# Mesoptier/ray-marching

Measured on AMD Instinct MI355X. Metric: Mpixels/s at 1920x1080, 256-step march, 32-node SDF, higher is better.
Workload: dtype f32; 1 GPU; 1920x1080, g32 (31 commands / 111 words), 256 max steps, 16 rays/px, RGBA32F out; camera=still, kernel=0, specialized_kernel=True, jit_from_disk_cache=True, frames_in_flight=4

## Files before the change

### ray-marching_amd/csrc/rm_jit.h

```cpp
#pragma once
#include <atomic>
#include <chrono>
#include <condition_variable>
#include <cstdio>
#include <cstdlib>
#include <cstring>
#include <dlfcn.h>
#include <sys/stat.h>
#include <unistd.h>
#include <map>
#include <memory>
#include <mutex>
#include <string>
#include <thread>
#include <vector>

#include "rm_device.h"
#include "rm_units.h"

namespace rmjit {

#include "generated/rm_jit_sources.inc"

constexpr uint32_t kMaxRecords = 255u;

struct Rtc {
    typedef struct _hiprtcProgram* Program;
    int (*CreateProgram)(Program*, const char*, const char*, int, const char* const*, const char* const*) = nullptr;
    int (*CompileProgram)(Program, int, const char* const*) = nullptr;
    int (*GetProgramLogSize)(Program, size_t*) = nullptr;
    int (*GetProgramLog)(Program, char*) = nullptr;
    int (*GetCodeSize)(Program, size_t*) = nullptr;
    int (*GetCode)(Program, char*) = nullptr;
// ... 36 lines not shown
        DestroyProgram = reinterpret_cast<decltype(DestroyProgram)>(sym("hiprtcDestroyProgram"));
        if (!all) { handle = nullptr; return; }
        Version = reinterpret_cast<decltype(Version)>(dlsym(handle, "hiprtcVersion"));
        int major = 0, minor = 0;
        if (Version) (void)Version(&major, &minor);
        Dl_info info;
        std::memset(&info, 0, sizeof info);
        (void)dladdr(reinterpret_cast<void*>(CreateProgram), &info);
        identity = std::string(info.dli_fname ? info.dli_fname : "?") + ":" + std::to_string(major) + "." + std::to_string(minor);
    }
};

inline std::string structure_key(const std::vector<RmRecord>& rec) {
    std::string k;
    k.reserve(rec.size() * 2);
    for (const RmRecord& r : rec) {
        k.push_back("PSBCLXM?"[RM_OP_KIND(r.op)]);
        k.push_back("pusixy??"[RM_OP_MODE(r.op)]);
        if (RM_OP_KIND(r.op) == RM_KIND_POP && RM_OP_MODE(r.op) == RM_MODE_SMOOTH && !(r.p[0] == r.p[0] && std::fabs(r.p[0]) < 1.0e30f)) k.push_back('!');
    }
    return k;
}

inline bool can_specialise(const std::vector<RmRecord>& rec) { return !rec.empty() && rec.size() <= kMaxRecords; }

inline int jit_knob(const char* name, int dflt) {
    const char* v = std::getenv(name);
    return v ? std::atoi(v) : dflt;
}

enum : int { PRUNE_NONE = 0, PRUNE_LATTICE = 1, PRUNE_BLEND = 2 };
enum : int { KERNEL_WITH_STATS = 0x100, PRUNE_KIND_MASK = 0xFF };

inline bool generate_scene_code(const std::vector<RmRecord>& rec, int prune, int T, std::string* out) {
    const int count_mode = (prune && T == 1) ? jit_knob("RM_JIT_PRUNE_STATS", 0) : 0;
    const char* counted = count_mode == 1 ? " n_eval += 1u;" : "";
    const int sched_every = T == 1 ? 4 : 2;
    const bool sub_tests = jit_knob("RM_JIT_SUB_TESTS", 1) != 0 && T == 1;
    const bool fence = T == 4;
    std::vector<RmUnit> units;
    if (prune == PRUNE_LATTICE && !rm_lattice_units(rec, &units)) return false;
    if (prune == PRUNE_BLEND && !rm_blend_units(rec, &units)) return false;
    std::vector<int> unit_at(rec.size(), -1);
    for (size_t u = 0; u < units.size(); u++) unit_at[(size_t)units[u].first] = (int)u;

    std::string s;
    char line[1024];
    s += "namespace rmk {\ntemplate <bool FAST>\n";
    if (T == 1) {
        s += "RM_DEV float map_scene_spec(LdsF lp, float qx, float qy, float qz, unsigned long long need, unsigned long long live, SqrtGuard& tiny, uint32_t& n_eval) {\n";
        if (prune) s += "    const float inf = __uint_as_float(0x7F800000u);\n";
        s += "    const float x0 = qx, y0 = qy, z0 = qz;\n";
    } else {
        s += "RM_DEV void map_scene_taps(LdsF lp, float cx, float cy, float cz, unsigned long long need, unsigned long long live, SqrtGuard& tiny, float (&f)[4]) {\n";
        if (prune) s += "    const float inf = __uint_as_float(0x7F800000u);\n";
        s += "    const float e = 0.0001f;\n";
        s += "    const float x0_0 = cx + e, x0_1 = cx - e, x0_2 = cx - e, x0_3 = cx + e;\n";
        s += "    const float y0_0 = cy - e, y0_1 = cy - e, y0_2 = cy + e, y0_3 = cy + e;\n";
        s += "    const float z0_0 = cz - e, z0_1 = cz + e, z0_2 = cz - e, z0_3 = cz + e;\n";
    }
    auto V = [&](int w, int t) { char b[32]; if (T == 1) std::snprintf(b, sizeof b, "v%d", w); else std::snprintf(b, sizeof b, "v%d_%d", w, t); return std::string(b); };
    auto P = [&](int c, int t) {
        char b[96];
        if (T == 1) std::snprintf(b, sizeof b, "x%d, y%d, z%d", c, c, c);
        else std::snprintf(b, sizeof b, "x%d_%d, y%d_%d, z%d_%d", c, t, c, t, c, t);
        return std::string(b);
    };
    auto leaf_fn = [](uint32_t kind) -> const char* {
        return kind == RM_KIND_SPHERE ? "spec_sphere<FAST>" : kind == RM_KIND_BOX ? "spec_box<FAST>" : kind == RM_KIND_CYLINDER ? "spec_cylinder<FAST>"
             : kind == RM_KIND_PLANE ? "spec_plane" : nullptr;
    };
    auto leaf_expr = [&](size_t i, int c, int t) {
        const uint32_t kind = RM_OP_KIND(rec[i].op);
        char b[256];
        if (kind == RM_KIND_PLANE) std::snprintf(b, sizeof b, "%s(lp + %u, %s)", leaf_fn(kind), (unsigned)i * 8u, P(c, t).c_str());
        else std::snprintf(b, sizeof b, "%s(lp + %u, %s, tiny)", leaf_fn(kind), (unsigned)i * 8u, P(c, t).c_str());
        return std::string(b);
// ... 2 lines not shown
    auto emit_smooth = [&](const char* decl, int w, unsigned koff, const std::vector<std::string>& a, const std::vector<std::string>& b, const char* ind) {
        if (T == 1) {
            std::snprintf(line, sizeof line, "%s%s%s = spec_smooth_union(lp + %u, %s, %s, live);\n", ind, decl, V(w, 0).c_str(), koff, a[0].c_str(), b[0].c_str());
            s += line;
            return;
        }
        if (decl[0]) {
            std::snprintf(line, sizeof line, "%sfloat %s, %s, %s, %s;\n", ind, V(w, 0).c_str(), V(w, 1).c_str(), V(w, 2).c_str(), V(w, 3).c_str());
            s += line;
        }
        std::snprintf(line, sizeof line,
                      "%s{ const float sa[4] = {%s, %s, %s, %s}, sb[4] = {%s, %s, %s, %s}; float so[4];\n"
                      "%s  spec_smooth_union4(lp + %u, sa, sb, live, so); %s = so[0]; %s = so[1]; %s = so[2]; %s = so[3]; }\n",
                      ind, a[0].c_str(), a[1].c_str(), a[2].c_str(), a[3].c_str(), b[0].c_str(), b[1].c_str(), b[2].c_str(), b[3].c_str(),
                      ind, koff, V(w, 0).c_str(), V(w, 1).c_str(), V(w, 2).c_str(), V(w, 3).c_str());
        s += line;
    };
    auto names = [&](int w) { std::vector<std::string> n; for (int t = 0; t < T; t++) n.push_back(V(w, t)); return n; };

    std::vector<int> stack;
    std::vector<int> pos;
    pos.push_back(0);
    int nv = 0, np = 0, leaves = 0;
    auto after_leaf = [&](bool is_plane) {
        if (fence && !is_plane) s += "    guard_fence(tiny);\n";
        if (sched_every > 0 && ++leaves % sched_every == 0) s += "    __builtin_amdgcn_sched_barrier(0);\n";
    };
    auto emit_plain = [&](size_t first, size_t last, const char* ind) -> bool {
        for (size_t i = first; i <= last; i++) {
            const uint32_t kind = RM_OP_KIND(rec[i].op), mode = RM_OP_MODE(rec[i].op);
            const unsigned off = (unsigned)i * 8u;
            if (kind == RM_KIND_MATERIAL) return false;
            if (kind == RM_KIND_XFORM) {
                const int c = pos.back();
                if ((mode & 1u) == 0u) {
                    const int n = ++np;
                    for (int t = 0; t < T; t++) {
                        char cx[24], cy[24], cz[24], nx[24], ny[24], nz[24];
                        auto nm = [&](char* b, char a, int q) { if (T == 1) std::snprintf(b, 24, "%c%d", a, q); else std::snprintf(b, 24, "%c%d_%d", a, q, t); };
                        nm(cx, 'x', c); nm(cy, 'y', c); nm(cz, 'z', c); nm(nx, 'x', n); nm(ny, 'y', n); nm(nz, 'z', n);
                        if (mode == RM_XF_T_PUSH)
                            std::snprintf(line, sizeof line, "%sconst float %s = %s - lp[%u], %s = %s - lp[%u], %s = %s - lp[%u];\n", ind, nx, cx, off, ny, cy, off + 1u, nz, cz, off + 2u);
                        else if (mode == RM_XF_R_PUSH)
                            std::snprintf(line, sizeof line, "%sfloat %s = %s, %s = %s, %s = %s; xf_rotate_conj(lp[%u], lp[%u], lp[%u], lp[%u], %s, %s, %s);\n",
                                          ind, nx, cx, ny, cy, nz, cz, off, off + 1u, off + 2u, off + 3u, nx, ny, nz);
                        else
                            std::snprintf(line, sizeof line, "%sconst float %s = %s / lp[%u], %s = %s / lp[%u], %s = %s / lp[%u];\n", ind, nx, cx, off, ny, cy, off, nz, cz, off);
                        s += line;
                    }
                    pos.push_back(n);
                } else {
                    if (pos.size() < 2 || stack.empty()) return false;
                    pos.pop_back();
                    if (mode == RM_XF_S_POP) {
                        const int a = stack.back(); stack.pop_back();
                        const int w = nv++;
                        for (int t = 0; t < T; t++) {
                            std::snprintf(line, sizeof line, "%sconst float %s = %s * lp[%u];\n", ind, V(w, t).c_str(), V(a, t).c_str(), off);
                            s += line;
                        }
                        stack.push_back(w);
                    }
                }
                continue;
            }
            const char* op = op_name(mode);
            if (kind == RM_KIND_POP) {
                if (stack.size() < 2 || mode == RM_MODE_PUSH) return false;
                const int b = stack.back(); stack.pop_back();
                const int a = stack.back(); stack.pop_back();
                const int w = nv++;
                if (mode == RM_MODE_SMOOTH) {
                    emit_smooth("const float ", w, off, names(a), names(b), ind);
                } else {
                    if (!op) return false;
                    for (int t = 0; t < T; t++) {
                        std::snprintf(line, sizeof line, "%sconst float %s = %s(%s, %s);\n", ind, V(w, t).c_str(), op, V(a, t).c_str(), V(b, t).c_str());
                        s += line;
                    }
                }
                stack.push_back(w);
                continue;
            }
            if (!leaf_fn(kind) || mode == RM_MODE_SMOOTH || (mode != RM_MODE_PUSH && !op)) return false;
            int a = -1;
            if (mode != RM_MODE_PUSH) {
                if (stack.empty()) return false;
                a = stack.back(); stack.pop_back();
            }
            const int w = nv++;
            for (int t = 0; t < T; t++) {
                if (mode == RM_MODE_PUSH) std::snprintf(line, sizeof line, "%sconst float %s = %s;%s\n", ind, V(w, t).c_str(), leaf_expr(i, pos.back(), t).c_str(), counted);
                else std::snprintf(line, sizeof line, "%sconst float %s = %s(%s, %s);%s\n", ind, V(w, t).c_str(), op, V(a, t).c_str(), leaf_expr(i, pos.back(), t).c_str(), counted);
                s += line;
            }
            stack.push_back(w);
            after_leaf(kind == RM_KIND_PLANE);
        }
        return true;
    };

    std::vector<int> group_first(units.size(), 0);
    if (jit_knob("RM_JIT_UNIT_GROUPS", 1) != 0) {
        auto flows = [&](size_t u) {
            const RmUnit& q = units[u];
            if (q.kind == RM_UNIT_OPAQUE || q.leaf < 0) return false;
            const uint32_t m = q.k_rec >= 0 ? (uint32_t)RM_MODE_SMOOTH : RM_OP_MODE(rec[(size_t)q.first].op);
            if (m == RM_MODE_PUSH || (m == RM_MODE_INTER && q.kind == RM_UNIT_LEAF)) return false;
            return true;
        };
        auto pushes = [&](size_t u) {
            const RmUnit& q = units[u];
            if (q.kind == RM_UNIT_OPAQUE || q.leaf < 0 || q.k_rec >= 0 || q.first != q.last) return false;
            return RM_OP_MODE(rec[(size_t)q.first].op) == RM_MODE_PUSH;
        };
        for (size_t u = 0; u < units.size();) {
            if (!flows(u) && !(pushes(u) && u + 1 < units.size() && flows(u + 1) && units[u + 1].first == units[u].last + 1)) { u++; continue; }
// ... 12 lines not shown
    int group_left = 0, group_value = -1;

    for (size_t i = 0; i < rec.size();) {
        const int ui = unit_at[i];
        if (ui < 0) {
            if (!emit_plain(i, i, "    ")) return false;
            i++;
            continue;
        }
        const RmUnit& u = units[(size_t)ui];
        const uint32_t kind = RM_OP_KIND(rec[i].op), mode = RM_OP_MODE(rec[i].op);
        const int c = pos.back();
        if (group_left == 0 && group_first[(size_t)ui] != 0) {
            const bool fresh = mode == RM_MODE_PUSH && u.k_rec < 0;
            if (!fresh && stack.empty()) return false;
            group_left = group_first[(size_t)ui];
            group_value = nv++;
            for (int t = 0; t < T; t++) {
                std::snprintf(line, sizeof line, "    float %s = %s;\n", V(group_value, t).c_str(), fresh ? "inf" : V(stack.back(), t).c_str());
                s += line;
            }
            uint32_t mask = 0u;
            for (int k = 0; k < group_left; k++) mask |= 1u << ((ui + k) & 31);
            std::snprintf(line, sizeof line, "    { const uint32_t wg = unit_word(need, %du);\n    if ((wg & 0x%xu) != 0u) {\n", ui, mask);
            s += line;
        }
        char guard[64];
        if (group_left != 0) std::snprintf(guard, sizeof guard, "unit_in_word(wg, %du)", ui);
        else std::snprintf(guard, sizeof guard, "unit_needed(need, %du)", ui);
        auto close_group = [&]() {
            if (group_left == 0 || --group_left != 0) return;
            for (int t = 0; t < T; t++) { std::snprintf(line, sizeof line, "        %s = %s;\n", V(group_value, t).c_str(), V(stack.back(), t).c_str()); s += line; }
            s += "    } }\n";
            stack.back() = group_value;
        };
        if (u.kind == RM_UNIT_OPAQUE) {
            if (stack.empty()) return false;
            const int a = stack.back();
            const int w = nv++;
            for (int t = 0; t < T; t++) { std::snprintf(line, sizeof line, "    float %s = %s;\n", V(w, t).c_str(), V(a, t).c_str()); s += line; }
            std::snprintf(line, sizeof line, "    if (unit_needed(need, %du)) {\n", ui);
            s += line;
            const size_t depth0 = stack.size();
            if (!emit_plain((size_t)u.first, (size_t)u.last, "        ") || stack.size() != depth0) return false;
            for (int t = 0; t < T; t++) { std::snprintf(line, sizeof line, "        %s = %s;\n", V(w, t).c_str(), V(stack.back(), t).c_str()); s += line; }
            s += "    }\n";
            stack.back() = w;
            i = (size_t)u.last + 1u;
            continue;
        }
        const bool with_smooth = u.k_rec >= 0;
        const uint32_t eff_mode = with_smooth ? (uint32_t)RM_MODE_SMOOTH : mode;
        int a = -1;
        if (eff_mode != RM_MODE_PUSH) {
            if (stack.empty()) return false;
            a = stack.back(); stack.pop_back();
        }
        const int w = nv++;
        const bool to_inf = eff_mode == RM_MODE_PUSH || (eff_mode == RM_MODE_INTER && u.kind == RM_UNIT_LEAF);
        for (int t = 0; t < T; t++) {
            if (to_inf) std::snprintf(line, sizeof line, "    float %s = inf;\n", V(w, t).c_str());
            else std::snprintf(line, sizeof line, "    float %s = %s;\n", V(w, t).c_str(), V(a, t).c_str());
            s += line;
        }
        std::snprintf(line, sizeof line, "    if (%s) {%s\n", guard, counted);
        s += line;
        const unsigned off = (unsigned)i * 8u;
        if (with_smooth) {
            std::vector<std::string> lv;
            for (int t = 0; t < T; t++) lv.push_back(leaf_expr(i, c, t));
            emit_smooth("", w, (unsigned)u.k_rec * 8u, names(a), lv, "        ");
        } else if (eff_mode == RM_MODE_SUB && sub_tests && (kind == RM_KIND_SPHERE || kind == RM_KIND_BOX)) {
            if (kind == RM_KIND_SPHERE)
                std::snprintf(line, sizeof line, "        const float a = spec_sphere_a(lp + %u, %s);\n        if (spec_sub_sphere_near(live, lp + %u, a, %s)) %s = vmax_negb(%s, spec_sphere_v<FAST>(lp + %u, a, tiny));\n",
                              off, P(c, 0).c_str(), off, V(a, 0).c_str(), V(w, 0).c_str(), V(a, 0).c_str(), off);
            else
                std::snprintf(line, sizeof line, "        const SpecBox b = spec_box_a(lp + %u, %s);\n        if (spec_sub_box_near(live, b.a, %s)) %s = vmax_negb(%s, spec_box_v<FAST>(b, tiny));\n",
                              off, P(c, 0).c_str(), V(a, 0).c_str(), V(w, 0).c_str(), V(a, 0).c_str());
            s += line;
        } else {
            const char* op = op_name(eff_mode);
            if (eff_mode != RM_MODE_PUSH && !op) return false;
            for (int t = 0; t < T; t++) {
                if (eff_mode == RM_MODE_PUSH) std::snprintf(line, sizeof line, "        %s = %s;\n", V(w, t).c_str(), leaf_expr(i, c, t).c_str());
                else std::snprintf(line, sizeof line, "        %s = %s(%s, %s);\n", V(w, t).c_str(), op, V(a, t).c_str(), leaf_expr(i, c, t).c_str());
                s += line;
            }
        }
        s += "    }\n";
        stack.push_back(w);
        after_leaf(false);
        close_group();
        i = (size_t)u.last + 1u;
    }
    if (stack.empty() || group_left != 0) return false;
    if (T == 1) {
        std::snprintf(line, sizeof line, "    return %s;\n}\n}  // namespace rmk\n", V(stack.back(), 0).c_str());
        s += line;
    } else {
        for (int t = 0; t < 4; t++) {
            std::snprintf(line, sizeof line, "    f[%d] = %s;\n", t, V(stack.back(), t).c_str());
            s += line;
        }
        s += "}\n}  // namespace rmk\n";
    }
    *out = std::move(s);
    return true;
}


inline bool generate_material_walk(const std::vector<RmRecord>& mrec, std::string* out) {
    std::string s;
    char line[768];
    s += "namespace rmk {\n";
    s += "template <bool FAST>\n";
    s += "RM_DEV uint32_t map_scene_material_spec(const RmRecord* __restrict__ mp, float qx, float qy, float qz, SqrtGuard& tiny) {\n";
    s += "    const float x0 = qx, y0 = qy, z0 = qz;\n";
    std::vector<int> stack, pos;
    pos.push_back(0);
    int nv = 0, np = 0, leaves = 0;
    for (size_t i = 0; i < mrec.size(); i++) {
        const uint32_t kind = RM_OP_KIND(mrec[i].op), mode = RM_OP_MODE(mrec[i].op);
        const unsigned r = (unsigned)i;
        if (kind == RM_KIND_MATERIAL) {
            if (stack.empty()) return false;
            const int a = stack.back(); stack.pop_back();
            const int w = nv++;
            std::snprintf(line, sizeof line, "    const float v%d = v%d; const uint32_t m%d = __float_as_uint(mp[%u].p[0]);\n", w, a, w, r);
            s += line;
            stack.push_back(w);
            continue;
// ... 74 lines not shown
            std::snprintf(an, sizeof an, "v%d", a); std::snprintf(am, sizeof am, "m%d", a); std::snprintf(bn, sizeof bn, "v%d", leaf);
            if (!combine(w, an, am, bn, "0u")) return false;
            stack.push_back(w);
        }
    }
    if (stack.empty()) return false;
    std::snprintf(line, sizeof line, "    return m%d;\n}\n}  // namespace rmk\n", stack.back());
    s += line;
    *out = std::move(s);
    return true;
}

inline const char* kernel_name() { return "rm_render_v5_spec"; }

inline bool structure_allows_bound_walk(const std::vector<RmRecord>& rec) {
    bool smooth = false;
    int spilled = 0, depth = 0;
    for (const RmRecord& r : rec) {
        const uint32_t kind = RM_OP_KIND(r.op);
        if (kind == RM_KIND_XFORM || kind == RM_KIND_MATERIAL) return false;
        smooth = smooth || RM_OP_MODE(r.op) == RM_MODE_SMOOTH || RM_OP_MODE(r.op) == RM_MODE_INTER || kind == RM_KIND_PLANE;
        if (kind == RM_KIND_POP) spilled--;
        else if (r.op & RM_OP_SPILL) spilled++;
        depth = spilled > depth ? spilled : depth;
    }
    return smooth && depth <= 1;
}

inline bool generate_source(const std::vector<RmRecord>& rec, const std::vector<RmRecord>& mrec, int wpt, int prune_kind, std::string* out,
                            bool* walk_generated = nullptr, bool* taps4_generated = nullptr, std::string* capped_out = nullptr) {
    const bool materials = !mrec.empty();
    const bool with_stats = (prune_kind & KERNEL_WITH_STATS) != 0;
    prune_kind &= PRUNE_KIND_MASK;
    std::string body, taps, walk;
    if (!generate_scene_code(rec, prune_kind, 1, &body)) return false;
    const bool walk_spec = materials && mrec.size() <= kMaxRecords && generate_material_walk(mrec, &walk);
    if (walk_generated) *walk_generated = walk_spec;
    const bool taps4 = generate_scene_code(rec, prune_kind, 4, &taps);
    if (taps4_generated) *taps4_generated = taps4;
    std::string s;
    s += "typedef unsigned char rm_rtc_u8;\ntypedef unsigned short rm_rtc_u16;\ntypedef unsigned int rm_rtc_u32;\n"
         "typedef unsigned long long rm_rtc_u64;\ntypedef int rm_rtc_i32;\ntypedef long long rm_rtc_i64;\n"
         "#define uint8_t rm_rtc_u8\n#define uint16_t rm_rtc_u16\n#define uint32_t rm_rtc_u32\n#define uint64_t rm_rtc_u64\n"
         "#define int32_t rm_rtc_i32\n#define int64_t rm_rtc_i64\n";
    s += "#define RM_JIT_TU 1\n";
    if (prune_kind == PRUNE_LATTICE) s += "#define RM_JIT_PRUNE_ON 1\n";
    if (prune_kind == PRUNE_BLEND) s += "#define RM_JIT_BLEND_PRUNE 1\n";
    if (taps4) s += "#define RM_JIT_TAPS4 1\n";
    if (walk_spec) s += "#define RM_JIT_MATERIAL_WALK 1\n";
    if (structure_allows_bound_walk(rec)) s += "#define RM_JIT_BOUND_WALK 1\n";
    if (!with_stats) s += "#define RM_NO_WAVE_STATS 1\n";
    s += "#include \"rm_kernel_v5.h\"\n";
    s += body;
    if (taps4) s += taps;
    if (walk_spec) s += walk;
    char line[512];
    int waves = prune_kind == PRUNE_BLEND ? 6 : 0;
    bool chain = !materials && taps4 && prune_kind != PRUNE_BLEND && !rec.empty();
    for (size_t i = 1; chain && i < rec.size(); i++) {
        const uint32_t kind = RM_OP_KIND(rec[i].op), mode = RM_OP_MODE(rec[i].op);
        chain = (kind == RM_KIND_SPHERE || kind == RM_KIND_BOX || kind == RM_KIND_CYLINDER || kind == RM_KIND_PLANE) && mode != RM_MODE_PUSH;
    }
    if (chain) waves = 7;
    const bool probe = capped_out && waves == 0 && prune_kind == PRUNE_LATTICE && !materials && jit_knob("RM_JIT_PROBE_CAP", 1) != 0;
    auto kernel_text = [&](int w) {
        std::string k;
        if (w > 0) {
            std::snprintf(line, sizeof line, "__attribute__((amdgpu_waves_per_eu(%d, %d)))\n", w, w);
            k += line;
        }
        std::snprintf(line, sizeof line,
                      "extern \"C\" __global__ __launch_bounds__(%d) void %s(RmLaunch L, rmk::V5Work work, uint32_t n_tiles, "
                      "uint32_t refill_min) {\n    rmk::rm_render_v5_body<rmk::ProgLds, true, %d, false, true, %s>(L, work, n_tiles, refill_min);\n}\n",
                      64 * wpt, kernel_name(), wpt, materials ? "true" : "false");
        k += line;
        return k;
    };
    if (capped_out) *capped_out = probe ? s + kernel_text(6) : std::string();
    s += kernel_text(waves);
    *out = std::move(s);
    return true;
}

struct CacheHeader {
    char magic[8];
    uint64_t bytes;
// ... 177 lines not shown
    bool material_walk = false;
    bool taps4 = false;
    bool from_cache = false;
    std::string cached_source;
    struct Loaded { void* module = nullptr; void* function = nullptr; };
    std::map<int, Loaded> loaded;
    void (*unload)(void* module, int device) = nullptr;

    State wait() {
        std::unique_lock<std::mutex> lk(m);
        cv.wait(lk, [&] { return state != COMPILING; });
        return state;
    }
    State peek() {
        std::lock_guard<std::mutex> lk(m);
        return state;
    }
    ~Entry() {
        if (unload)
            for (auto& kv : loaded)
                if (kv.second.module) unload(kv.second.module, kv.first);
    }
};

class Cache {
public:
    static constexpr size_t kMaxEntries = 256;

    static Cache& get() {
        static Cache* c = new Cache;
        return *c;
    }
    std::shared_ptr<Entry> request(const std::vector<RmRecord>& rec, const std::vector<RmRecord>& mrec, int wpt, int prune) {
        static const char* const knobs[] = {"RM_JIT_PRUNE_STATS", "RM_JIT_SUB_TESTS", "RM_JIT_UNIT_GROUPS", "RM_JIT_PROBE_CAP"};
        std::string knob_key;
        for (const char* name : knobs)
            if (const char* v = std::getenv(name)) knob_key += std::string("|") + name + "=" + v;
        const std::string key = std::to_string(wpt) + ((prune & PRUNE_KIND_MASK) == PRUNE_LATTICE ? "p" : (prune & PRUNE_KIND_MASK) == PRUNE_BLEND ? "b" : "") +
                                ((prune & KERNEL_WITH_STATS) ? "s" : "") + ":" + structure_key(rec) +
                                (mrec.empty() ? "" : "|m:" + structure_key(mrec)) + knob_key;
        std::unique_lock<std::mutex> lk(m_);
        auto it = entries_.find(key);
        if (it != entries_.end()) return it->second;
        if (entries_.size() >= kMaxEntries) {
            for (auto j = entries_.begin(); j != entries_.end();)
                j = (j->second.use_count() == 1 && j->second->peek() != Entry::COMPILING) ? entries_.erase(j) : ++j;
        }
        auto e = std::make_shared<Entry>();
        entries_[key] = e;
        Job job;
        job.entry = e;
        if (!generate_source(rec, mrec, wpt, prune, &job.source, &e->material_walk, &e->taps4, &job.capped)) {
            e->state = Entry::FAILED;
            e->log = "program structure could not be turned into code";
            return e;
        }
        queue_.push_back(std::move(job));
        if (!worker_.joinable()) {
            worker_ = std::thread([this] { run(); });
            std::atexit([] { Cache::get().shutdown(); });
        }
        lk.unlock();
        cv_.notify_one();
        return e;
    }
    size_t size() {
        std::lock_guard<std::mutex> lk(m_);
// ... 61 lines not shown
```

### ray-marching_amd/csrc/rm_kernel_v5.h

```cpp
#pragma once
#include "rm_interp.h"
#include "rm_lds_layout.h"

namespace rmk {

typedef const __attribute__((address_space(3))) float* LdsF;
RM_DEV LdsF lds_vector_base(const void* generic_lds_ptr) {
    const uint32_t s = (uint32_t)(__SIZE_TYPE__)(const __attribute__((address_space(3))) void*)generic_lds_ptr;
    uint32_t v;
    asm("v_mov_b32 %0, %1" : "=v"(v) : "s"(s));
    return (LdsF)(__SIZE_TYPE__)v;
}
template <bool FAST>
RM_DEV float map_scene_spec(LdsF lp, float qx, float qy, float qz, unsigned long long need, unsigned long long live, SqrtGuard& tiny, uint32_t& n_eval);
#ifdef RM_JIT_MATERIAL_WALK
template <bool FAST>
RM_DEV uint32_t map_scene_material_spec(const RmRecord* __restrict__ mp, float qx, float qy, float qz, SqrtGuard& tiny);
#endif
#ifdef RM_JIT_TAPS4
template <bool FAST>
RM_DEV void map_scene_taps(LdsF lp, float cx, float cy, float cz, unsigned long long need, unsigned long long live, SqrtGuard& tiny, float (&f)[4]);
#endif

constexpr float kPruneAbs = 4.0e-6f;
RM_DEV float anchor_reach(float px, float py, float pz, float sd, float prune_scale) {
    return __builtin_fabsf(sd) * 1.00001f + kPruneAbs * (prune_scale + ((__builtin_fabsf(px) + __builtin_fabsf(py)) + __builtin_fabsf(pz)));
}
RM_DEV float anchor_thr_base(float thr_base, float qx, float qy, float qz, float ax, float ay, float az, float aT) {
    const float l1 = (__builtin_fabsf(qx - ax) + __builtin_fabsf(qy - ay)) + __builtin_fabsf(qz - az);
    const float t = __builtin_fmaf(l1, 1.00001f, aT);
    return t < thr_base ? t : thr_base;
}
#if defined(RM_JIT_PRUNE_ON) || !defined(RM_JIT_TU)
#define RM_PRUNE_PLUMBING 1
#endif

#define RM_DPP(old, src, ctrl) ((uint32_t)__builtin_amdgcn_update_dpp((int)(old), (int)(src), (ctrl), 0xF, 0xF, false))
RM_DEV uint32_t wave_max_u32(uint32_t v) {
    uint32_t t;
    t = RM_DPP(0u, v, 0xB1); v = t > v ? t : v;
    t = RM_DPP(0u, v, 0x4E); v = t > v ? t : v;
    t = RM_DPP(0u, v, 0x141); v = t > v ? t : v;
    t = RM_DPP(0u, v, 0x140); v = t > v ? t : v;
    t = (uint32_t)__builtin_amdgcn_update_dpp(0, (int)v, 0x142, 0xA, 0xF, false); v = t > v ? t : v;
    t = (uint32_t)__builtin_amdgcn_update_dpp(0, (int)v, 0x143, 0xC, 0xF, false); v = t > v ? t : v;
    return (uint32_t)__builtin_amdgcn_readlane((int)v, 63);
}
// ... 131 lines not shown
    }
    return k;
}
RM_DEV void stage_tree(uint32_t* ltree, const RmRecord* __restrict__ tree, uint32_t n_tree, uint32_t tid, uint32_t n_threads) {
    const uint32_t* src = reinterpret_cast<const uint32_t*>(tree);
    for (uint32_t k = tid; k < 5u * n_tree; k += n_threads) {
        const uint32_t f = k / n_tree, r = k - f * n_tree;
        ltree[k] = src[8u * r + 1u + f];
    }
}
#undef RM_DPP

#if !defined(RM_JIT_TU)
__global__ __launch_bounds__(64) void rm_selftest_wave_kernel(const float* in, float* out, uint32_t n_waves) {
    const uint32_t i = blockIdx.x * 64u + threadIdx.x;
    const float x = in[i];
    out[i] = __uint_as_float(wave_max_u32(__float_as_uint(x)));
    out[64u * n_waves + i] = wave_exclusive_min(x);
}
#endif

RM_DEV bool unit_needed(unsigned long long need, uint32_t u) {
    uint32_t w = (uint32_t)(need >> (u & 32u));
    asm volatile("" : "+s"(w));
    return ((w >> (u & 31u)) & 1u) != 0u;
}

RM_DEV uint32_t unit_word(unsigned long long need, uint32_t u) {
    uint32_t w = (uint32_t)(need >> (u & 32u));
    asm volatile("" : "+s"(w));
    return w;
}
RM_DEV bool unit_in_word(uint32_t w, uint32_t u) { return ((w >> (u & 31u)) & 1u) != 0u; }

typedef float lds_f4 __attribute__((ext_vector_type(4)));
typedef float lds_f2 __attribute__((ext_vector_type(2)));
RM_DEV lds_f4 lds_load4(LdsF r) { return *reinterpret_cast<const __attribute__((address_space(3))) lds_f4*>(r); }
RM_DEV lds_f2 lds_load2(LdsF r) { return *reinterpret_cast<const __attribute__((address_space(3))) lds_f2*>(r); }
RM_DEV float spec_sphere_a(LdsF r, float qx, float qy, float qz) {
    const lds_f4 p = lds_load4(r);
    const float dx = qx - p.x, dy = qy - p.y, dz = qz - p.z;
    return (dx * dx + dy * dy) + dz * dz;
}
template <bool FAST>
RM_DEV float spec_sphere_v(LdsF r, float a, SqrtGuard& tiny) { return sqrt_sel<FAST>(a, tiny) - r[3]; }
RM_DEV bool spec_sub_sphere_near(unsigned long long live, LdsF r, float a, float acc) {
    const float rk = r[4];
    return ((__builtin_amdgcn_ballot_w64(!(a > rk * rk)) | __builtin_amdgcn_ballot_w64(!(acc >= 0.0f))) & live) != 0ull;
}
RM_DEV bool spec_sub_box_near(unsigned long long live, float a, float acc) {
    return ((__builtin_amdgcn_ballot_w64(!(a > 0.0f)) | __builtin_amdgcn_ballot_w64(!(acc >= 0.0f))) & live) != 0ull;
}
struct SpecBox { float qx, qy, qz, a; };
RM_DEV SpecBox spec_box_a(LdsF r, float px, float py, float pz) {
    const lds_f4 c = lds_load4(r);
    const lds_f2 h = lds_load2(r + 4);
    SpecBox b;
    b.qx = __builtin_fabsf(px - c.x) - c.w;
    b.qy = __builtin_fabsf(py - c.y) - h.x;
    b.qz = __builtin_fabsf(pz - c.z) - h.y;
    const float mx = fmax_(b.qx, 0.0f), my = fmax_(b.qy, 0.0f), mz = fmax_(b.qz, 0.0f);
    b.a = (mx * mx + my * my) + mz * mz;
    return b;
}
template <bool FAST>
RM_DEV float spec_box_v(const SpecBox& b, SqrtGuard& tiny) {
// ... 355 lines not shown
            prog.load(i, op, p);
        }
    };
    const float bound_scale = prune_scale + L.smooth_slack;
    const LdsF lprog_v = lds_vector_base(lprog);
    uint32_t n_eval = 0u;
    const uint32_t* lunits = lprog + 8u * L.n_rec;
    auto units_needed = [&](float x, float y, float z, float thr, float extra_margin, bool is_live, unsigned long long live_mask) -> unsigned long long {
        if constexpr (SPEC) {
#if defined(RM_JIT_PRUNE_ON)
            return wave_cull_lattice(lunits, L.n_grp, x, y, z, thr, is_live, live_mask);
#elif defined(RM_JIT_BLEND_PRUNE)
            return wave_cull_blend(lunits, L.n_grp, L.unit_kmax, x, y, z, extra_margin, prune_scale, is_live, live_mask);
#else
            return ~0ull;
#endif
        } else if constexpr (LOOP == 2 || LOOP == 4) {
            return wave_cull_lattice(lunits, L.n_grp, x, y, z, thr, is_live, live_mask);
        } else if constexpr (LOOP == 1 || LOOP == 3) {
            return ~0ull;
        } else if constexpr (PROG_IN_LDS) {
            if ((L.flags & 8u) == 0u) return ~0ull;
            if (L.unit_mode == RM_UNITS_LATTICE) return wave_cull_lattice(lunits, L.n_grp, x, y, z, thr, is_live, live_mask);
            return wave_cull_blend(lunits, L.n_grp, L.unit_kmax, x, y, z, extra_margin, prune_scale, is_live, live_mask);
        } else {
            return ~0ull;
        }
    };
    auto eval_scene = [&](float x, float y, float z, float thr, bool is_live, unsigned long long live_mask) -> float {
        float qx[1] = {x}, qy[1] = {y}, qz[1] = {z}, v[1];
        SqrtGuard tiny;
        if constexpr (SPEC) {
            const unsigned long long need = units_needed(x, y, z, thr, 0.0f, is_live, live_mask);
            v[0] = map_scene_spec<true>(lprog_v, x, y, z, need, live_mask, tiny, n_eval);
            if (tiny.any_bad()) {
                asm volatile("");
                uint32_t again = 0u;
                v[0] = map_scene_spec<false>(lprog_v, x, y, z, need, live_mask, tiny, again);
            }
        } else if (LOOP == 1 || LOOP == 2 || (LOOP == 0 && (L.flags & 4u))) {
            const unsigned long long need = units_needed(x, y, z, thr, 0.0f, is_live, live_mask);
            const bool masked = LOOP == 0 ? (PROG_IN_LDS && (L.flags & 8u) != 0u) : LOOP == 2;
#ifdef RM_INTERP_STATS
            n_eval += (uint32_t)__builtin_popcountll(masked ? need : (L.n_rec >= 64u ? ~0ull : (1ull << L.n_rec) - 1ull));
#endif
            v[0] = map_scene_chain<true>(prog, L.n_rec, x, y, z, need, masked, tiny);
            if (tiny.any_bad()) v[0] = map_scene_chain<false>(prog, L.n_rec, x, y, z, need, masked, tiny);
        } else if (LOOP == 3 || LOOP == 4 || (LOOP == 0 && !EXT)) {
            const bool masked = LOOP == 0 ? (PROG_IN_LDS && (L.flags & 8u) != 0u) : LOOP == 4;
            if (masked) {
                const unsigned long long need = units_needed(x, y, z, thr, 0.0f, is_live, live_mask);
                const TreeKeep k = tree_keep(lunits + 8u * L.n_grp, L.n_rec, need);
#ifdef RM_INTERP_STATS
                n_eval += (uint32_t)(__builtin_popcountll(k.keep0) + __builtin_popcountll(k.keep1));
#endif
                v[0] = map_scene_tree_masked<true>(prog, spill, x, y, z, k.keep0, k.keep1, k.push0, k.push1, tiny);
                if (tiny.any_bad()) v[0] = map_scene_tree_masked<false>(prog, spill, x, y, z, k.keep0, k.keep1, k.push0, k.push1, tiny);
            } else {
                v[0] = map_scene_tree<true>(prog, L.n_rec, spill, x, y, z, tiny);
                if (tiny.any_bad()) v[0] = map_scene_tree<false>(prog, L.n_rec, spill, x, y, z, tiny);
            }
        } else if (PROG_IN_LDS && (L.flags & 8u)) {
            const unsigned long long need = units_needed(x, y, z, thr, 0.0f, is_live, live_mask);
            const uint32_t* ranges = lunits + 7u * L.n_grp;
            v[0] = map_scene_units<true, EXT>(prog, ranges, spill, x, y, z, need, tiny, L.value_spill_depth);
            if (tiny.any_bad())
                v[0] = map_scene_units<false, EXT>(prog, ranges, spill, x, y, z, need, tiny, L.value_spill_depth);
        } else {
            map_scene_multi<1, true, Prog, EXT>(prog, L.n_rec, spill, L.max_dist, qx, qy, qz, v, tiny, L.value_spill_depth);
            if (tiny.any_bad()) map_scene_multi<1, false, Prog, EXT>(prog, L.n_rec, spill, L.max_dist, qx, qy, qz, v, tiny, L.value_spill_depth);
        }
// ... 315 lines not shown
                                const float4 al = L.materials[rmat[s * 64u + p]];
                                cr = al.x * code; cg = al.y * code; cb = al.z * code;
                            }
                        }
                    } else if (code > -2.5f) {
                        const float g = 0.2f * (-1.0f - code);
                        cr = 0.1f + g; cg = 0.1f + g; cb = 0.2f + g;
                    } else {
                        cr = 0.0f; cg = 0.0f; cb = 0.0f;
                    }
                    tr += sqrt_sel<FAST, true>(cr, guard);
                    tg += sqrt_sel<FAST, true>(cg, guard);
                    tb += sqrt_sel<FAST, true>(cb, guard);
                }
            };
            float tr, tg, tb;
            SqrtGuard gamma_guard;
            sum_samples(TrueTag(), tr, tg, tb, gamma_guard);
            if (gamma_guard.bad()) sum_samples(FalseTag(), tr, tg, tb, gamma_guard);
            store_pixel(L, blockIdx.z, (size_t)py * L.W + px, tr / 16.0f, tg / 16.0f, tb / 16.0f);
        }
    }
    if (work.measured && tid == 0u) {
        const unsigned long long dt = __builtin_amdgcn_s_memrealtime() - tile_t0;
        work.measured[(size_t)blockIdx.z * n_tiles + tile] = dt > 0xFFFFFFFFull ? 0xFFFFFFFFu : (dt == 0ull ? 1u : (uint32_t)dt);
    }
    __syncthreads();
  }
    if (L.stats && lane == 0u) {
        unsigned long long* st = L.stats + 4ull * (((size_t)blockIdx.z * gridDim.x + blockIdx.x) * WPT + wave);
        st[0] = t_start;
        st[1] = __builtin_amdgcn_s_memrealtime();
        st[2] = ((unsigned long long)n_tiles_done << 32) | n_iter;
        st[3] = ((unsigned long long)(n_eval != 0u ? n_eval : n_prod) << 32) | n_live;
    }
}

template <class Prog, bool PROG_IN_LDS, int WPT, bool EXT>
__global__ __launch_bounds__(64 * WPT) void rm_render_v5(RmLaunch L, V5Work work, uint32_t n_tiles, uint32_t refill_min) {
    rm_render_v5_body<Prog, PROG_IN_LDS, WPT, EXT, false, EXT>(L, work, n_tiles, refill_min);
}
template <int WPT, int LOOP>
__global__ __launch_bounds__(64 * WPT) __attribute__((amdgpu_waves_per_eu(6, 8)))
void rm_render_v5_lean(RmLaunch L, V5Work work, uint32_t n_tiles, uint32_t refill_min) {
    rm_render_v5_body<ProgLds, true, WPT, false, false, false, LOOP>(L, work, n_tiles, refill_min);
}

constexpr uint32_t V5_PRE_TILES = 4u;
constexpr uint32_t V5_PRE_BLOCK = 32u;
static_assert(V5_PRE_BLOCK >= 1u && V5_PRE_BLOCK <= 64u, "one wave classifies the block, lane = tile");

#if !defined(RM_JIT_TU)
RM_DEV bool rect_cone_v5(const float* m_proj, const float* m_view, const V4& ro, const float (&px)[2], const float (&py)[2], const float (&ox)[2],
                         const float (&oy)[2], float noise, float (&cone_out)[4], float (&corner)[4][3]) {
    float cx = 0.0f, cy = 0.0f, cz = 0.0f, ex[4], ey[4], ez[4], inv_hi = 0.0f;
#pragma unroll
    for (uint32_t c = 0; c < 4u; c++) {
        gen_ray_unnormalized_at(m_proj, m_view, ro, px[c & 1u], py[c >> 1], ox[c & 1u], oy[c >> 1], ex[c], ey[c], ez[c]);
        corner[c][0] = ex[c]; corner[c][1] = ey[c]; corner[c][2] = ez[c];
        const float inv = __builtin_amdgcn_rsqf(__builtin_fmaf(ez[c], ez[c], __builtin_fmaf(ey[c], ey[c], ex[c] * ex[c])));
        ex[c] *= inv; ey[c] *= inv; ez[c] *= inv;
        inv_hi = fmax_(inv_hi, inv);
        cx += ex[c]; cy += ey[c]; cz += ez[c];
    }
    unit_dir(cx, cy, cz);
    float rho2 = 0.0f;
#pragma unroll
// ... 597 lines not shown
```

Baseline: 7435 Mpixels/s.

## Add JIT single-unit fast path that evaluates only the one needed SDF unit

```diff
diff --git a/ray-marching_amd/csrc/rm_jit.h b/ray-marching_amd/csrc/rm_jit.h
--- a/ray-marching_amd/csrc/rm_jit.h
+++ b/ray-marching_amd/csrc/rm_jit.h
@@ -1,4 +1,5 @@
 #pragma once
+#include <algorithm>
 #include <atomic>
 #include <chrono>
 #include <condition_variable>
@@ -101,7 +102,7 @@
 enum : int { PRUNE_NONE = 0, PRUNE_LATTICE = 1, PRUNE_BLEND = 2 };
 enum : int { KERNEL_WITH_STATS = 0x100, PRUNE_KIND_MASK = 0xFF };
 
-inline bool generate_scene_code(const std::vector<RmRecord>& rec, int prune, int T, std::string* out) {
+inline bool generate_scene_code(const std::vector<RmRecord>& rec, int prune, int T, std::string* out, std::string* walk_out = nullptr) {
     const int count_mode = (prune && T == 1) ? jit_knob("RM_JIT_PRUNE_STATS", 0) : 0;
     const char* counted = count_mode == 1 ? " n_eval += 1u;" : "";
     const int sched_every = T == 1 ? 4 : 2;
@@ -112,6 +113,36 @@
     if (prune == PRUNE_BLEND && !rm_blend_units(rec, &units)) return false;
     std::vector<int> unit_at(rec.size(), -1);
     for (size_t u = 0; u < units.size(); u++) unit_at[(size_t)units[u].first] = (int)u;
+
+    struct One { int state; float c; std::string expr; };
+    struct Sym { float cst; std::map<int, One> one; };
+    const float kInf = INFINITY;
+    const int walk_knob = jit_knob("RM_JIT_UNIT_WALK", 1);
+    bool walk_ok = walk_out != nullptr && T == 1 && prune == PRUNE_LATTICE && walk_knob != 0 && units.size() >= 2 && units.size() <= 32;
+    for (size_t u = 0; walk_ok && u < units.size(); u++) walk_ok = units[u].first == (int)u && units[u].last == (int)u;
+    std::map<int, Sym> sym;
+    auto cname = [&](float c) { return std::string(c > 0.0f ? "inf" : "-inf"); };
+    auto fold = [&](uint32_t mode, const One& l, const One& r) -> One {
+        if (l.state == 2 || r.state == 2 || (l.state == 1 && r.state == 1)) return One{2, 0.0f, ""};
+        const char* fn = mode == RM_MODE_UNION ? "vmin" : mode == RM_MODE_SUB ? "vmax_negb" : "fmax_";
+        if (l.state == 0 && r.state == 0)
+            return One{0, mode == RM_MODE_UNION ? std::fmin(l.c, r.c) : mode == RM_MODE_SUB ? std::fmax(l.c, -r.c) : std::fmax(l.c, r.c), ""};
+        if (l.state == 0) {
+            if (mode == RM_MODE_UNION ? l.c < 0.0f : l.c > 0.0f) return One{0, l.c, ""};
+            return One{1, 0.0f, std::string(fn) + "(" + cname(l.c) + ", " + r.expr + ")"};
+        }
+        if (mode == RM_MODE_UNION ? r.c < 0.0f : mode == RM_MODE_SUB ? r.c < 0.0f : r.c > 0.0f) return One{0, mode == RM_MODE_UNION ? r.c : kInf, ""};
+        return One{1, 0.0f, std::string(fn) + "(" + l.expr + ", " + cname(r.c) + ")"};
+    };
+    auto sym_pop = [&](uint32_t mode, int a, int b, int w) {
+        if (!walk_ok) return;
+        const Sym &A = sym[a], &B = sym[b];
+        Sym W;
+        W.cst = fold(mode, One{0, A.cst, ""}, One{0, B.cst, ""}).c;
+        for (const auto& kv : A.one) W.one[kv.first] = fold(mode, kv.second, One{0, B.cst, ""});
+        for (const auto& kv : B.one) W.one[kv.first] = fold(mode, One{0, A.cst, ""}, kv.second);
+        sym[w] = std::move(W);
+    };
 
     std::string s;
     char line[1024];
@@ -180,6 +211,7 @@
             const unsigned off = (unsigned)i * 8u;
             if (kind == RM_KIND_MATERIAL) return false;
             if (kind == RM_KIND_XFORM) {
+                walk_ok = false;
                 const int c = pos.back();
                 if ((mode & 1u) == 0u) {
                     const int n = ++np;
@@ -219,9 +251,11 @@
                 const int a = stack.back(); stack.pop_back();
                 const int w = nv++;
                 if (mode == RM_MODE_SMOOTH) {
+                    walk_ok = false;
                     emit_smooth("const float ", w, off, names(a), names(b), ind);
                 } else {
                     if (!op) return false;
+                    sym_pop(mode, a, b, w);
                     for (int t = 0; t < T; t++) {
                         std::snprintf(line, sizeof line, "%sconst float %s = %s(%s, %s);\n", ind, V(w, t).c_str(), op, V(a, t).c_str(), V(b, t).c_str());
                         s += line;
@@ -231,6 +265,7 @@
                 continue;
             }
             if (!leaf_fn(kind) || mode == RM_MODE_SMOOTH || (mode != RM_MODE_PUSH && !op)) return false;
+            walk_ok = false;
             int a = -1;
             if (mode != RM_MODE_PUSH) {
                 if (stack.empty()) return false;
@@ -309,10 +344,12 @@
             if (group_left == 0 || --group_left != 0) return;
             for (int t = 0; t < T; t++) { std::snprintf(line, sizeof line, "        %s = %s;\n", V(group_value, t).c_str(), V(stack.back(), t).c_str()); s += line; }
             s += "    } }\n";
+            if (walk_ok) sym[group_value] = sym[stack.back()];
             stack.back() = group_value;
         };
         if (u.kind == RM_UNIT_OPAQUE) {
             if (stack.empty()) return false;
+            walk_ok = false;
             const int a = stack.back();
             const int w = nv++;
             for (int t = 0; t < T; t++) { std::snprintf(line, sizeof line, "    float %s = %s;\n", V(w, t).c_str(), V(a, t).c_str()); s += line; }
@@ -335,6 +372,16 @@
         }
         const int w = nv++;
         const bool to_inf = eff_mode == RM_MODE_PUSH || (eff_mode == RM_MODE_INTER && u.kind == RM_UNIT_LEAF);
+        if (with_smooth) walk_ok = false;
+        if (walk_ok) {
+            Sym W;
+            W.cst = to_inf ? kInf : sym[a].cst;
+            if (!to_inf) W.one = sym[a].one;
+            if (eff_mode == RM_MODE_PUSH) W.one[ui] = One{1, 0.0f, "@"};
+            else W.one[ui] = fold(eff_mode, One{0, sym[a].cst, ""}, One{1, 0.0f, "@"});
+            if (eff_mode == RM_MODE_SUB && W.one[ui].state != 0) W.one[ui] = One{2, 0.0f, ""};
+            sym[w] = std::move(W);
+        }
         for (int t = 0; t < T; t++) {
             if (to_inf) std::snprintf(line, sizeof line, "    float %s = inf;\n", V(w, t).c_str());
             else std::snprintf(line, sizeof line, "    float %s = %s;\n", V(w, t).c_str(), V(a, t).c_str());
@@ -374,6 +421,57 @@
     if (T == 1) {
         std::snprintf(line, sizeof line, "    return %s;\n}\n}  // namespace rmk\n", V(stack.back(), 0).c_str());
         s += line;
+        if (walk_out) walk_out->clear();
+        if (walk_ok) {
+            struct Class { std::string key, action; uint32_t mask; bool open; };
+            std::vector<Class> classes;
+            const Sym& R = sym[stack.back()];
+            const char* count = count_mode == 1 || count_mode == 5 ? " n_eval += 1u;" : "";
+            for (size_t u = 0; u < units.size(); u++) {
+                const auto it = R.one.find((int)u);
+                const One o = it == R.one.end() ? One{0, R.cst, ""} : it->second;
+                Class c;
+                c.mask = 1u << u;
+                c.open = o.state == 2;
+                if (o.state == 0) {
+                    c.key = "c" + cname(o.c);
+                    c.action = std::string(count) + " return " + cname(o.c) + ";";
+                } else if (o.state == 1) {
+                    const uint32_t kind = RM_OP_KIND(rec[(size_t)units[u].first].op);
+                    std::string call = std::string(leaf_fn(kind)) + "(r, qx, qy, qz, tiny)", e = o.expr;
+                    e.replace(e.find('@'), 1, call);
+                    if (o.expr == "vmin(inf, @)") e = "vmin_pinf(" + call + ")";
+                    c.key = std::to_string(kind) + "|" + o.expr;
+                    c.action = std::string(count) + " return " + e + ";";
+                } else {
+                    c.key = "open";
+                }
+                size_t k = 0;
+                while (k < classes.size() && classes[k].key != c.key) k++;
+                if (k == classes.size()) classes.push_back(c);
+                else classes[k].mask |= c.mask;
+            }
+            std::stable_sort(classes.begin(), classes.end(), [](const Class& a, const Class& b) {
+                if (a.open != b.open) return b.open;
+                return __builtin_popcount(a.mask) > __builtin_popcount(b.mask);
+            });
+            std::string w;
+            w += "namespace rmk {\ntemplate <bool FAST>\n";
+            w += "RM_DEV float map_scene_walk(LdsF lp, float qx, float qy, float qz, unsigned long long need, unsigned long long live, SqrtGuard& tiny, uint32_t& n_eval) {\n";
+            w += "    const uint32_t m = (uint32_t)need;\n";
+            w += "    uint32_t n_units;\n    asm volatile(\"s_bcnt1_i32_b32 %0, %1\" : \"=s\"(n_units) : \"s\"(m) : \"scc\");\n";
+            w += "    if (n_units == 1u) {  // exactly one unit: s_bcnt1_i32_b32, s_cmp_lg_u32, branch\n";
+            w += "        const float inf = __uint_as_float(0x7F800000u);\n";
+            w += "        const LdsF r = lp + 8u * (uint32_t)__builtin_ctz(m);\n";
+            for (size_t k = 0; k < classes.size(); k++) {
+                if (classes[k].open) break;
+                if (k + 1 < classes.size()) std::snprintf(line, sizeof line, "        if ((m & 0x%xu) != 0u) {%s }\n", classes[k].mask, classes[k].action.c_str());
+                else std::snprintf(line, sizeof line, "       %s\n", classes[k].action.c_str());
+                w += line;
+            }
+            w += "    }\n    return map_scene_spec<FAST>(lp, qx, qy, qz, need, live, tiny, n_eval);\n}\n}  // namespace rmk\n";
+            *walk_out = std::move(w);
+        }
     } else {
         for (int t = 0; t < 4; t++) {
             std::snprintf(line, sizeof line, "    f[%d] = %s;\n", t, V(stack.back(), t).c_str());
@@ -514,8 +612,8 @@
     const bool materials = !mrec.empty();
     const bool with_stats = (prune_kind & KERNEL_WITH_STATS) != 0;
     prune_kind &= PRUNE_KIND_MASK;
-    std::string body, taps, walk;
-    if (!generate_scene_code(rec, prune_kind, 1, &body)) return false;
+    std::string body, taps, walk, unit_walk;
+    if (!generate_scene_code(rec, prune_kind, 1, &body, &unit_walk)) return false;
     const bool walk_spec = materials && mrec.size() <= kMaxRecords && generate_material_walk(mrec, &walk);
     if (walk_generated) *walk_generated = walk_spec;
     const bool taps4 = generate_scene_code(rec, prune_kind, 4, &taps);
@@ -532,8 +630,11 @@
     if (walk_spec) s += "#define RM_JIT_MATERIAL_WALK 1\n";
     if (structure_allows_bound_walk(rec)) s += "#define RM_JIT_BOUND_WALK 1\n";
     if (!with_stats) s += "#define RM_NO_WAVE_STATS 1\n";
+    if (!unit_walk.empty()) s += "#define RM_JIT_UNIT_WALK 1\n";
+    if (prune_kind && jit_knob("RM_JIT_PRUNE_STATS", 0) == 5) s += "#define RM_JIT_WALK_COUNTER 1\n";
     s += "#include \"rm_kernel_v5.h\"\n";
     s += body;
+    s += unit_walk;
     if (taps4) s += taps;
     if (walk_spec) s += walk;
     char line[512];
@@ -777,7 +878,7 @@
         return *c;
     }
     std::shared_ptr<Entry> request(const std::vector<RmRecord>& rec, const std::vector<RmRecord>& mrec, int wpt, int prune) {
-        static const char* const knobs[] = {"RM_JIT_PRUNE_STATS", "RM_JIT_SUB_TESTS", "RM_JIT_UNIT_GROUPS", "RM_JIT_PROBE_CAP"};
+        static const char* const knobs[] = {"RM_JIT_PRUNE_STATS", "RM_JIT_SUB_TESTS", "RM_JIT_UNIT_GROUPS", "RM_JIT_UNIT_WALK", "RM_JIT_PROBE_CAP"};
         std::string knob_key;
         for (const char* name : knobs)
             if (const char* v = std::getenv(name)) knob_key += std::string("|") + name + "=" + v;
diff --git a/ray-marching_amd/csrc/rm_kernel_v5.h b/ray-marching_amd/csrc/rm_kernel_v5.h
--- a/ray-marching_amd/csrc/rm_kernel_v5.h
+++ b/ray-marching_amd/csrc/rm_kernel_v5.h
@@ -13,6 +13,13 @@
 }
 template <bool FAST>
 RM_DEV float map_scene_spec(LdsF lp, float qx, float qy, float qz, unsigned long long need, unsigned long long live, SqrtGuard& tiny, uint32_t& n_eval);
+#ifdef RM_JIT_UNIT_WALK
+template <bool FAST>
+RM_DEV float map_scene_walk(LdsF lp, float qx, float qy, float qz, unsigned long long need, unsigned long long live, SqrtGuard& tiny, uint32_t& n_eval);
+#define RM_MAP_SCENE_STEP map_scene_walk
+#else
+#define RM_MAP_SCENE_STEP map_scene_spec
+#endif
 #ifdef RM_JIT_MATERIAL_WALK
 template <bool FAST>
 RM_DEV uint32_t map_scene_material_spec(const RmRecord* __restrict__ mp, float qx, float qy, float qz, SqrtGuard& tiny);
@@ -210,6 +217,11 @@
     return w;
 }
 RM_DEV bool unit_in_word(uint32_t w, uint32_t u) { return ((w >> (u & 31u)) & 1u) != 0u; }
+RM_DEV float vmin_pinf(float b) {
+    float r;
+    asm("v_min_f32 %0, 0x7f800000, %1" : "=v"(r) : "v"(b));
+    return r;
+}
 
 typedef float lds_f4 __attribute__((ext_vector_type(4)));
 typedef float lds_f2 __attribute__((ext_vector_type(2)));
@@ -631,11 +643,11 @@
         SqrtGuard tiny;
         if constexpr (SPEC) {
             const unsigned long long need = units_needed(x, y, z, thr, 0.0f, is_live, live_mask);
-            v[0] = map_scene_spec<true>(lprog_v, x, y, z, need, live_mask, tiny, n_eval);
+            v[0] = RM_MAP_SCENE_STEP<true>(lprog_v, x, y, z, need, live_mask, tiny, n_eval);
             if (tiny.any_bad()) {
                 asm volatile("");
                 uint32_t again = 0u;
-                v[0] = map_scene_spec<false>(lprog_v, x, y, z, need, live_mask, tiny, again);
+                v[0] = RM_MAP_SCENE_STEP<false>(lprog_v, x, y, z, need, live_mask, tiny, again);
             }
         } else if (LOOP == 1 || LOOP == 2 || (LOOP == 0 && (L.flags & 4u))) {
             const unsigned long long need = units_needed(x, y, z, thr, 0.0f, is_live, live_mask);
@@ -1017,7 +1029,11 @@
         st[0] = t_start;
         st[1] = __builtin_amdgcn_s_memrealtime();
         st[2] = ((unsigned long long)n_tiles_done << 32) | n_iter;
+#ifdef RM_JIT_WALK_COUNTER
+        st[3] = ((unsigned long long)n_eval << 32) | n_live;
+#else
         st[3] = ((unsigned long long)(n_eval != 0u ? n_eval : n_prod) << 32) | n_live;
+#endif
     }
 }
 
```

Result: faster. 7601 Mpixels/s, median of 6 (+2.2%).
